# Chris10M/Ev2Hands

Measured on AMD Instinct MI355X. Metric: event-windows/sec at B=256 N=2048 (f16x2), higher is better.
Workload: dtype f32 (each f32 operand split into 2 fp16 planes with per-window power-of-two range scaling, 3 plane products per MAC on the f16 MFMA, f32 accumulate); 1 GPU; TEHNet.forward+MANO both hands, B=256/GPU N=2048 C=4 fp32, E-clouds, random-init 342-key checkpoint, synthetic MANO-shaped assets; global_batch=256, points=2048, channels=4, precision=f16x2, forwards_in_flight=1, world_size_seen=1, parallelism=batch-shard x1

## Files before the change

### ev2hands_amd/csrc/sa_mlp_bf16.hip

```cpp
#include <algorithm>
#include <cmath>
#include <cstdlib>
#include <type_traits>
#include "planes.hpp"
#include "ev2hands_hip.h"

namespace {

struct SaBP {
    const float* P1; int ldp;
    const float4* pts4;
    const float4* ctr4;
    const int32_t* gidx;
    const float4* W1x;
    const char* W2s; const float* b2;
    const char* W3s; const float* b3;
    float* out; int ldo;
    int B, Npts, S, K;
    int S_total, s_off;
    int nblk;
    const int32_t* cnt; int cnt_ld;
    float u2, u3;
    int per_xcd;
    const float* p1_scale; const unsigned* p1_amax;
    float w1x_norm, dmax, w2_norm, b2_max;
    unsigned* out_amax;
    const int32_t* nn_idx; const float* nn_w; int N;
    int ncols; int relu_out; float* out_cm; size_t out_cm_stride;
    const float* feat; int ldf; const float* W1f; int ldw1f; const float* b1; int nfeat;
    const unsigned* feat_amax; float w1f_norm, b1_max, u1f, u1x;
    float a1f, a1x, a1b;
    int spg;
    float* xyz_out; int xyz_ld;
    int t_bf16, out_bf16;
    float* row16_scale; float w3_norm, b3_max;
};

#ifdef EV2H_SAB_TIMELINE
__device__ long long g_sab_timeline[256];
#define STAMP(i) do { if (dbgw && strip == dbg_strip) g_sab_timeline[(i)] = __builtin_amdgcn_s_memtime(); } while (0)
#else
#define STAMP(i) do { } while (0)
#endif
constexpr int SAB_WAVES = 8;
constexpr int SAB_THREADS = SAB_WAVES * 64;

// ... 5 lines not shown
    static constexpr int REM = C2 % 32;
    static constexpr int M_LAST = REM == 0 ? 2 : (REM <= 16 ? 1 : 2);
    static constexpr int C2P = 32 * (T2 - 1) + 16 * M_LAST;
    static constexpr int T3 = C3 / 32;
    static constexpr int NC1 = C1 / 32;
    static constexpr int RS2 = NPL * 64 + 16;
    static constexpr int RS3 = NPL * C2P * 2 + 16;
    static constexpr int TB2 = T2 * 32 * RS2;
    static constexpr int TB3 = 32 * RS3;
    static constexpr int SB2W = F16 ? SAB_WAVES * T2 * 32 * 4 : 0;
    static constexpr int RSA = (NS == 3) ? 112 : 80;
    static constexpr int W1B = (NS == 1 || NS == 4) ? C1 * 32 : F16 ? C1 * RSA + SAB_WAVES * C1 * 4 : C1 * RSA + C1 * 4;
    static constexpr int REC_SLOTS = 64;
    static constexpr int REC = F16 ? REC_SLOTS * 4 : 0;
    static constexpr int SMALL_NOREC = W1B + T2 * 32 * 4 + 16 + SB2W;
    static constexpr int SMALL = SMALL_NOREC + REC;
    static constexpr int tile_bytes(int cpt, int upt) { return ((cpt * TB2 > upt * TB3 ? cpt * TB2 : upt * TB3) + 1023) / 1024 * 1024; }
    static constexpr bool fits(int n) { return NC1 % n == 0 && T3 % n == 0 && 2 * tile_bytes(n, n) + SMALL <= 158 * 1024; }
    static constexpr int CPT = fits(2) ? 2 : 1, UPT = CPT;
    static constexpr int TILE = tile_bytes(CPT, UPT);
    static constexpr int LDS_BYTES = 2 * TILE + SMALL;
    static constexpr int RES_W = (NC1 * TB2 + T3 * TB3 + 1023) / 1024 * 1024;
    static constexpr int RES_LDS_BYTES = RES_W + SMALL;
    static constexpr bool FITS_RESIDENT = RES_LDS_BYTES <= 160 * 1024 && C1 >= 64;
    static constexpr bool PACK4 = (NS == 2) && REM >= 1 && REM <= 4;
};

template <int C1, int C2, int C3, int NS, bool RES, int MODE>
constexpr int sab_min_waves() {
    return (NS == 4 && RES && MODE == 3 && 2 * SaBCfg<C1, C2, C3, NS>::RES_LDS_BYTES <= 160 * 1024) ? 4 : 2;
}
template <int C1, int C2, int C3, int NS, bool RES, int MODE = 0>
__global__ __launch_bounds__(SAB_THREADS, (sab_min_waves<C1, C2, C3, NS, RES, MODE>())) void sa_mlp_max_bf16_kernel(SaBP p) {
    constexpr int WV = SAB_WAVES;
    constexpr bool ROWS = MODE == 1 || MODE == 2, DIRECT = MODE == 2;
    static_assert(!(RES && ROWS), "the row-output variants stream their tiles");
    constexpr bool L1M = (NS == 1 || NS == 4) && !ROWS;
    constexpr bool L1F = (NS == 2 || NS == 3) && MODE == 3;
    constexpr bool L2PIPE = !ROWS && (NS == 1 || NS == 4) && (C1 / 32) % 2 == 0;
    constexpr bool H2FUSE = NS != 3;
    constexpr bool FRAG_PIPE = (NS != 3);
    using Cfg = SaBCfg<C1, C2, C3, NS>;
    using PL = Planes<NS>;
    constexpr int NPL = Cfg::NPL;
    constexpr bool F16 = Cfg::F16;
    constexpr int T2 = Cfg::T2, T3 = Cfg::T3, NC1 = Cfg::NC1, RS2 = Cfg::RS2, RS3 = Cfg::RS3, C2P = Cfg::C2P;
// ... 62 lines not shown
            }
        } else {
            for (int i = tid; i < C1; i += WV * 64) {
                const float4 w = p.W1x[i];
                float* d = reinterpret_cast<float*>(sW1xT) + (i >> 2) * 12 + (i & 3);
                d[0] = w.x; d[4] = w.y; d[8] = w.z;
            }
        }
    }
    for (int i = tid; i < T2 * 32; i += WV * 64) sb2[i] = p.b2[i] / p.u2;
    float* sbw = F16 ? reinterpret_cast<float*>(smem + WBYTES + Cfg::W1B + T2 * 32 * 4 + 16) + wave * (T2 * 32) : sb2;

    auto dma_tile = [&](const char* src, char* dst, int bytes) {
        for (int off = wave * 1024; off < bytes; off += WV * 1024) {
            if (off + lane * 16 < bytes)
                __builtin_amdgcn_global_load_lds((const __attribute__((address_space(1))) void*)(src + off + lane * 16),
                                                 (__attribute__((address_space(3))) void*)(dst + off), 16, 0, 0);
        }
    };
    constexpr int CPT = RES ? 1 : Cfg::CPT, UPT = RES ? 1 : Cfg::UPT;
    auto dma_w2 = [&](int step, char* dst) { dma_tile(p.W2s + (size_t)step * CPT * Cfg::TB2, dst, CPT * Cfg::TB2); };
    auto dma_w3 = [&](int step, char* dst) { dma_tile(p.W3s + (size_t)step * UPT * Cfg::TB3, dst, UPT * Cfg::TB3); };

    int buf = 0;
    if constexpr (RES && F16) {
        if (tid < Cfg::REC_SLOTS) reinterpret_cast<unsigned*>(smem + WBYTES + Cfg::SMALL_NOREC)[tid] = 0u;
    }
    if constexpr (RES) {
        dma_tile(p.W2s, smem, NC1 * Cfg::TB2);
        dma_tile(p.W3s, smem + NC1 * Cfg::TB2, T3 * Cfg::TB3);
    } else {
        dma_w2(0, wt0);
    }
    asm volatile("s_waitcnt vmcnt(0)" ::: "memory");
    __syncthreads();

    const int xcd = blockIdx.x & 7, slot = blockIdx.x >> 3, nbx = p.nblk >> 3;
    const int g_end = RES ? min(ngroups, (xcd + 1) * p.per_xcd) : ngroups;
  const int spg = (RES || ROWS) ? 1 : max(1, __builtin_amdgcn_readfirstlane(p.spg)), sw = wave % spg;
  for (int g = (RES ? xcd * p.per_xcd + slot * WV : (spg > 1 ? L * (WV / spg) + wave / spg : L * WV)) + wave * (RES || spg == 1); RES ? g < g_end : true;
       g += nbx * WV) {
    const bool valid = g < ngroups;
    const int gg = valid ? g : ngroups - 1;
    const int b = gg / p.S;
    const size_t gf = ROWS ? (size_t)gg : (size_t)b * p.S_total + p.s_off + (gg - b * p.S);
    float mrun[T3];
#pragma unroll
    for (int u = 0; u < T3; ++u) mrun[u] = -INFINITY;

    float4 ctr = make_float4(0.f, 0.f, 0.f, 0.f);
    const int32_t* gi = nullptr;
    if constexpr (!ROWS) { ctr = p.ctr4[gf]; gi = p.gidx + gf * p.K + sw * 32; }
    const int row0 = ROWS ? (gg - b * p.S) * 32 : 0;
    unsigned am = 0u;
    constexpr bool C2ONE = NS == 4 && !ROWS;
    float s1 = 1.f, c2 = p.u2, c3 = C2ONE ? p.u3 * p.u2 : p.u3;
    float so = 1.f;
    float b1s_f = 1.f, b1s_x = 1.f, b1s_b = 1.f;
    const bool fform = fmode || (L1M && hasfeat);
    if constexpr (F16) {
        if (fform && p.feat_amax) {
            const float bnd = __fmaf_rn(p.w1f_norm, __uint_as_float(p.feat_amax[b]), p.b1_max) + p.w1x_norm * p.dmax;
            s1 = f16x2_scale(__float_as_uint(bnd));
            float s2 = f16x2_scale(__float_as_uint(__fmaf_rn(p.w2_norm, bnd, p.b2_max)));
            if constexpr (C2ONE) { s1 = fminf(s1, p.u2 * s2); s2 = s1 * pow2_inverse(p.u2); }
            c2 = p.u2 * s2 * pow2_inverse(s1);
            c3 = p.u3 * pow2_inverse(s2);
        } else if (!fform && p.p1_amax) {
            float a1 = __uint_as_float(p.p1_amax[b]);
            if constexpr (DIRECT) {
                if (NS == 4 && p.t_bf16) s1 = p.row16_scale[b];
                else { s1 = f16x2_scale(p.p1_amax[b]); a1 *= s1; }
            }
            else s1 = p.p1_scale[b];
            const float inv_s1 = pow2_inverse(s1);
            const float bh1 = a1 + s1 * (p.w1x_norm * p.dmax);
            const float bh2 = __fmaf_rn(p.w2_norm, bh1 * inv_s1, p.b2_max);
            float s2 = f16x2_scale(__float_as_uint(bh2));
            c2 = p.u2 * s2 * inv_s1;
            c3 = p.u3 * pow2_inverse(s2);
            if constexpr (C2ONE) {
                s2 = s1 * pow2_inverse(p.u2);
                c3 = (s2 * bh2 <= 65504.f) ? p.u3 * pow2_inverse(s2) : __uint_as_float(0x7fc00000u);
            }
        }
        s1 = __uint_as_float(__builtin_amdgcn_readfirstlane(__float_as_uint(s1)));
        c2 = __uint_as_float(__builtin_amdgcn_readfirstlane(__float_as_uint(c2)));
        c3 = __uint_as_float(__builtin_amdgcn_readfirstlane(__float_as_uint(c3)));
        if constexpr (ROWS && NS == 4) {
            if (p.out_bf16) {
                const float bound2 = 32768.f * (c3 / p.u3);
                so = f16x2_scale(__float_as_uint(__fmaf_rn(p.w3_norm, bound2, p.b3_max)));
                so = __uint_as_float(__builtin_amdgcn_readfirstlane(__float_as_uint(so)));
                if (lane == 0 && valid && row0 == 0) p.row16_scale[b] = so;
            }
        }
        for (int i = lane; i < T2 * 32; i += 64) sbw[i] = sb2[i] * s1;
        if constexpr (L1F) {
            if (fmode) for (int i = lane; i < C1; i += 64) sb1w[i] = p.b1[i] * s1;
        }
        if constexpr (L1M) { b1s_f = s1 * p.a1f; b1s_x = s1 * p.a1x; b1s_b = s1 * p.a1b; }
    }
    int my_strips = ROWS ? 1 : p.K >> 5;
    if (!ROWS && p.cnt) my_strips = min(my_strips, max(1, (p.cnt[gf * p.cnt_ld] + 31) >> 5));
    if (spg > 1) my_strips = (valid && sw < my_strips) ? 1 : 0;
    int nstrips = my_strips;
    if constexpr (!RES && !ROWS) {
        int* s_strips = reinterpret_cast<int*>(smem + WBYTES + Cfg::W1B + T2 * 32 * 4);
        if (tid == 0) *s_strips = 1;
        __syncthreads();
        if (lane == 0) atomicMax(s_strips, my_strips);
        __syncthreads();
        nstrips = *s_strips;
    }

#ifdef EV2H_SAB_TIMELINE
    const bool dbgw = (blockIdx.x == 300 && tid == 0);
    const int dbg_strip = nstrips > 1 ? 1 : 0;
#endif
    constexpr bool XPF = !ROWS && NS != 3;
    f32x4 raw[4];
    int idx_cur = 0, idx_nxt = 0;
    float4 q_cur = make_float4(0.f, 0.f, 0.f, 0.f), f0_cur = q_cur, f1_cur = q_cur;
    if constexpr (XPF) {
        idx_cur = gi[l31];
        q_cur = p.pts4[(size_t)b * p.Npts + idx_cur];
        if (hasfeat) {
            const float4* fr = reinterpret_cast<const float4*>(p.feat + ((size_t)b * p.Npts + idx_cur) * p.ldf);
            f0_cur = fr[0]; f1_cur = fr[1];
        }
    }
    for (int strip = 0; strip < nstrips; ++strip) {
        STAMP(0);
        if constexpr (!RES) {
            if (strip >= my_strips) {
                for (int c = 0; c < NC1; ++c) {
                    char* nxt = buf ? wt0 : wt1;
                    if (c % CPT == 0) { if (c + CPT < NC1) dma_w2(c / CPT + 1, nxt); else dma_w3(0, nxt); }
                    if (c % CPT == CPT - 1) { asm volatile("s_waitcnt vmcnt(0)" ::: "memory"); __syncthreads(); buf ^= 1; }
                }
                for (int u = 0; u < T3; ++u) {
                    char* nxt = buf ? wt0 : wt1;
                    if (u % UPT == 0) { if (u + UPT < T3) dma_w3(u / UPT + 1, nxt); else if (strip + 1 < nstrips) dma_w2(0, nxt); }
                    if (u % UPT == UPT - 1) { asm volatile("s_waitcnt vmcnt(0)" ::: "memory"); __syncthreads(); buf ^= 1; }
                }
                continue;
            }
        }
        float dx = 0.f, dy = 0.f, dz = 0.f;
        auto qi = [&](int j4) { return 2 * j4 + half; };
        const float4* prow = nullptr;
        const float4* trow[3] = {nullptr, nullptr, nullptr};
        float tw[3] = {0.f, 0.f, 0.f};
        u32x4 b1f = {0u, 0u, 0u, 0u};
        u32x4 b1g = {0u, 0u, 0u, 0u};
        float cj = 1.f;
        f32x4 trw[ROWS ? 3 : 1][4];
        auto fetch = [&](int c) {
#pragma unroll
            for (int j = 0; j < ((ROWS && !DIRECT) ? 3 : 1); ++j)
#pragma unroll
                for (int j4 = 0; j4 < 4; ++j4) {
                    if constexpr ((NS == 1 || NS == 4) && DIRECT) {
                        if (p.t_bf16) {
                            const uint2 h = *reinterpret_cast<const uint2*>(reinterpret_cast<const char*>(trow[j]) + (size_t)(c * 32 + 4 * qi(j4)) * 2);
                            if constexpr (NS == 1) {
// ... 15 lines not shown
#pragma unroll
                for (int e = 0; e < 4; ++e)
                    raw[j4][e] = DIRECT ? ((F16 && !(NS == 4 && p.t_bf16)) ? trw[0][j4][e] * s1 : trw[0][j4][e])
                                        : __fmaf_rn(tw[2], trw[ROWS ? 2 : 0][j4][e], __fmaf_rn(tw[1], trw[ROWS ? 1 : 0][j4][e], __fmul_rn(tw[0], trw[0][j4][e])));
        };
        if constexpr (DIRECT) {
            trow[0] = ((NS == 1 || NS == 4) && p.t_bf16)
                          ? reinterpret_cast<const float4*>(reinterpret_cast<const char*>(p.P1) + ((size_t)b * p.N + min(row0 + l31, p.N - 1)) * p.ldp * 2)
                          : reinterpret_cast<const float4*>(p.P1 + ((size_t)b * p.N + min(row0 + l31, p.N - 1)) * p.ldp);
            fetch(0);
            blend();
        } else if constexpr (ROWS) {
            const size_t gr = ((size_t)b * p.N + min(row0 + l31, p.N - 1)) * 3;
#pragma unroll
            for (int j = 0; j < 3; ++j) {
                trow[j] = reinterpret_cast<const float4*>(p.P1 + ((size_t)b * p.Npts + p.nn_idx[gr + j]) * p.ldp);
                tw[j] = p.nn_w[gr + j];
            }
            fetch(0);
            blend();
        } else {
            const int idx = XPF ? idx_cur : gi[strip * 32 + l31];
            const float4 q = XPF ? q_cur : p.pts4[(size_t)b * p.Npts + idx];
            if constexpr (XPF) idx_nxt = (strip + 1 < my_strips) ? gi[(strip + 1) * 32 + l31] : idx_cur;
            dx = __fsub_rn(q.x, ctr.x); dy = __fsub_rn(q.y, ctr.y); dz = __fsub_rn(q.z, ctr.z);
            if constexpr (F16 && !L1M) { if (!fmode) { dx *= s1; dy *= s1; dz *= s1; } }
            if (fmode) {
                if constexpr (L1F && NS == 3) {
                    const float4* fr = reinterpret_cast<const float4*>(p.feat + ((size_t)b * p.Npts + idx) * p.ldf);
                    const float4 fa = fr[0], fb = fr[1];
                    const float v[8] = {fa.x, fa.y, fa.z, fa.w, fb.x, dx, dy, dz};
#pragma unroll
                    for (int w = 0; w < 4; ++w) {
                        unsigned o[3];
                        split_planes<3>(v[2 * w], v[2 * w + 1], o);
                        b1f[w] = half ? o[1] : o[0];
                        b1g[w] = half ? o[2] : o[0];
                    }
                }
                if constexpr (L1F && F16) {
                    float v[8] = {f0_cur.x, f0_cur.y, f0_cur.z, f0_cur.w, f1_cur.x, dx, dy, dz};
                    const float af = fmaxf(fmaxf(fmaxf(fabsf(v[0]), fabsf(v[1])), fmaxf(fabsf(v[2]), fabsf(v[3]))), fabsf(v[4]));
                    const float ax = fmaxf(fmaxf(fabsf(v[5]), fabsf(v[6])), fabsf(v[7]));
                    const float kap = fminf(f16x2_scale(__float_as_uint(af)) * (1.f / p.u1f), f16x2_scale(__float_as_uint(ax)) * (1.f / p.u1x));
                    const float sgf = kap * p.u1f, sgx = kap * p.u1x;
                    cj = s1 * pow2_inverse(kap);
#pragma unroll
                    for (int j = 0; j < 5; ++j) v[j] *= sgf;
#pragma unroll
                    for (int j = 5; j < 8; ++j) v[j] *= sgx;
#pragma unroll
                    for (int w = 0; w < 4; ++w) {
                        unsigned o[2];
                        split_planes<2>(v[2 * w], v[2 * w + 1], o);
                        b1f[w] = half ? o[1] : o[0];
                    }
                }
            } else if constexpr (L1M) {
                float f[8];
#pragma unroll
                for (int j = 0; j < 8; ++j) f[j] = 0.f;
                if (hasfeat) {
                    f[0] = f0_cur.x; f[1] = f0_cur.y; f[2] = f0_cur.z; f[3] = f0_cur.w; f[4] = f1_cur.x;
                    if constexpr (F16) {
#pragma unroll
                        for (int j = 0; j < 5; ++j) f[j] *= b1s_f;
                    }
                } else {
                    prow = reinterpret_cast<const float4*>(p.P1 + ((size_t)b * p.Npts + idx) * p.ldp);
                    if (strip == 0) {
#pragma unroll
                        for (int j4 = 0; j4 < 4; ++j4) raw[j4] = *reinterpret_cast<const f32x4*>(prow + qi(j4));
                    }
                }
                auto lo_of = [](float x) {
                    if constexpr (F16) return x - (float)(_Float16)x;
                    else return x - __uint_as_float(__builtin_bit_cast(unsigned, __builtin_convertvector(f32x2{x, 0.f}, bf16x2)) << 16);
                };
                const float ex = F16 ? dx * b1s_x : dx, ey = F16 ? dy * b1s_x : dy, ez = F16 ? dz * b1s_x : dz;
                const float va[8] = {f[0], f[1], f[2], f[3], f[4], lo_of(ex), lo_of(ey), lo_of(ez)};
                const float vb[8] = {ex, ey, ez, F16 ? (hasfeat ? b1s_b : 0.f) : 1.f, lo_of(f[0]), lo_of(f[1]), lo_of(f[2]), lo_of(f[3])};
#pragma unroll
                for (int w = 0; w < 4; ++w) {
                    unsigned o[1];
                    split_planes<NS>(half ? vb[2 * w] : va[2 * w], half ? vb[2 * w + 1] : va[2 * w + 1], o);
                    b1f[w] = o[0];
                }
            } else {
                prow = reinterpret_cast<const float4*>(p.P1 + ((size_t)b * p.Npts + idx) * p.ldp);
                if (!XPF || strip == 0) {
#pragma unroll
                    for (int j4 = 0; j4 < 4; ++j4) raw[j4] = *reinterpret_cast<const f32x4*>(prow + qi(j4));
                }
            }
        }
        auto layer1 = [&](int c) {
            f32x16 acc;
            if constexpr (L1F && NS == 3) {
#pragma unroll
                for (int q = 0; q < 4; ++q) {
                    const f32x4 bv = *reinterpret_cast<const f32x4*>(sb1w + 32 * c + 8 * q + 4 * half);
#pragma unroll
                    for (int e = 0; e < 4; ++e) acc[4 * q + e] = bv[e];
                }
                const char* ar = smem + WBYTES + (32 * c + l31) * Cfg::RSA + half * 16;
                const u32x4 a0 = *reinterpret_cast<const u32x4*>(ar), a1 = *reinterpret_cast<const u32x4*>(ar + 32), a2 = *reinterpret_cast<const u32x4*>(ar + 64);
                acc = mfma_planes<3>(a2, b1g, acc);
                acc = mfma_planes<3>(a1, b1f, acc);
                return mfma_planes<3>(a0, b1f, acc);
            } else if constexpr (L1F) {
#pragma unroll
                for (int r = 0; r < 16; ++r) acc[r] = 0.f;
                const char* ar = smem + WBYTES + (32 * c + l31) * Cfg::RSA + half * 16;
// ... 111 lines not shown
            if constexpr (FRAG_PIPE) ld2(0, fa[0][0], fa[0][1]);
#pragma unroll
            for (int pr = 0; pr < T2; ++pr) {
                const int m0 = (2 * pr) / T2, t0 = (2 * pr) % T2, m1 = (2 * pr + 1) / T2, t1 = (2 * pr + 1) % T2;
                if constexpr (FRAG_PIPE) {
                    if (pr + 1 < T2) ld2(pr + 1, fa[(pr + 1) & 1][0], fa[(pr + 1) & 1][1]);
                    __builtin_amdgcn_sched_barrier(0);
                } else {
                    ld2(pr, fa[pr & 1][0], fa[pr & 1][1]);
                }
                u32x4 (&a0)[NPL] = fa[pr & 1][0];
                u32x4 (&a1)[NPL] = fa[pr & 1][1];
#pragma unroll
                for (int j = 0; j < PL::NPROD; ++j) {
                    if (!(Cfg::PACK4 && t0 == T2 - 1 && PL::A[j] == 1)) h2[t0] = mfma_planes<NS>(a0[PL::A[j]], bp[m0][PL::B[j]], h2[t0]);
                    if (!(Cfg::PACK4 && t1 == T2 - 1 && PL::A[j] == 1)) h2[t1] = mfma_planes<NS>(a1[PL::A[j]], bp[m1][PL::B[j]], h2[t1]);
                }
                if constexpr (FRAG_PIPE) __builtin_amdgcn_sched_barrier(0);
                between(pr);
            }
        };
        auto l2_dma = [&](int c) {
            if constexpr (!RES) {
                char* nxt = buf ? wt0 : wt1;
                if (c % CPT == 0) { if (c + CPT < NC1) dma_w2(c / CPT + 1, nxt); else dma_w3(0, nxt); }
            }
        };
        auto l2_sync = [&](int c) {
            STAMP(4 + 4 * c);
            if constexpr (!RES) {
                if (c % CPT == CPT - 1) {
                    asm volatile("s_waitcnt vmcnt(0)" ::: "memory");
                    __syncthreads();
                    buf ^= 1;
                }
            }
            STAMP(5 + 4 * c);
        };
        u32x4 bpA[2][NPL];
        if constexpr (!L2PIPE) {
#pragma unroll 1
            for (int c = 0; c < NC1; ++c) {
                STAMP(2 + 4 * c);
                char* cur = RES ? smem + c * Cfg::TB2 : (buf ? wt1 : wt0) + (c % CPT) * Cfg::TB2;
                l2_dma(c);
#pragma unroll
                for (int j4 = 0; j4 < 4; ++j4) finish_slice(c, j4, bpA);
                if constexpr (ROWS) {
                    if (c + 1 < NC1) fetch(c + 1);
                } else if (!L1M && !fmode && c + 1 < NC1) {
#pragma unroll
                    for (int j4 = 0; j4 < 4; ++j4) raw[j4] = *reinterpret_cast<const f32x4*>(prow + (c + 1) * 8 + qi(j4));
                }
                STAMP(3 + 4 * c);
                mfma_groups(cur, bpA, [](int) {});
                if constexpr (ROWS) {
                    if (c + 1 < NC1) blend();
                }
                if constexpr (L1F) {
                    if (fmode && c + 1 < NC1) d1 = layer1(c + 1);
                }
                if constexpr (L1M) {
                    if (c + 1 < NC1) {
                        d1 = layer1(c + 1);
                        if (!hasfeat && c + 2 < NC1) {
#pragma unroll
                            for (int j4 = 0; j4 < 4; ++j4) raw[j4] = *reinterpret_cast<const f32x4*>(prow + (c + 2) * 8 + qi(j4));
                        }
                    }
                }
                l2_sync(c);
            }
        } else {
            u32x4 bpB[2][NPL];
            const bool vtab = !L1M && !fmode;
#pragma unroll
            for (int j4 = 0; j4 < 4; ++j4) {
                finish_slice(0, j4, bpA);
                if (vtab) raw[j4] = *reinterpret_cast<const f32x4*>(prow + 8 + qi(j4));
            }
            auto l2_step = [&](int c, u32x4 (&bc)[2][NPL], u32x4 (&bn)[2][NPL]) {
                STAMP(2 + 4 * c);
                char* cur = RES ? smem + c * Cfg::TB2 : (buf ? wt1 : wt0) + (c % CPT) * Cfg::TB2;
                l2_dma(c);
                const bool more = c + 1 < NC1;
                if (more) {
                    if constexpr (L1F) { if (fmode) d1 = layer1(c + 1); }
                    if constexpr (L1M) {
                        d1 = layer1(c + 1);
                        if (!hasfeat && c + 2 < NC1) {
#pragma unroll
                            for (int j4 = 0; j4 < 4; ++j4) raw[j4] = *reinterpret_cast<const f32x4*>(prow + (c + 2) * 8 + qi(j4));
                        }
                    }
                }
                STAMP(3 + 4 * c);
                mfma_groups(cur, bc, [&](int pr) {
                    if (more) {
#pragma unroll
                        for (int j4 = 0; j4 < 4; ++j4) {
                            if (j4 * T2 / 4 == pr) {
                                __builtin_amdgcn_sched_barrier(0);
                                finish_slice(c + 1, j4, bn);
                                if (vtab && c + 2 < NC1) raw[j4] = *reinterpret_cast<const f32x4*>(prow + (c + 2) * 8 + qi(j4));
                                __builtin_amdgcn_sched_barrier(0);
                            }
                        }
                    }
                });
                l2_sync(c);
            };
#pragma unroll 1
            for (int c = 0; c < NC1; c += 2) {
                l2_step(c, bpA, bpB);
                l2_step(c + 1, bpB, bpA);
            }
        }

        STAMP(38);
        if constexpr (XPF) {
            if (strip + 1 < my_strips) {
                q_cur = p.pts4[(size_t)b * p.Npts + idx_nxt];
                if (hasfeat) {
                    const float4* fr = reinterpret_cast<const float4*>(p.feat + ((size_t)b * p.Npts + idx_nxt) * p.ldf);
                    f0_cur = fr[0]; f1_cur = fr[1];
                } else {
                    const float4* pn = reinterpret_cast<const float4*>(p.P1 + ((size_t)b * p.Npts + idx_nxt) * p.ldp);
#pragma unroll
                    for (int j4 = 0; j4 < 4; ++j4) raw[j4] = *reinterpret_cast<const f32x4*>(pn + qi(j4));
                }
                idx_cur = idx_nxt;
            }
        }
        if constexpr (Cfg::PACK4) {
#pragma unroll
            for (int r = 0; r < 4; ++r) { h2[T2 - 1][r] += h2[T2 - 1][r + 4]; h2[T2 - 1][r + 4] = 0.f; }
        }
        u32x4 h2p[NPL][T2][2];
        auto split_half = [&](int t, int m) {
#pragma unroll
            for (int k = 4 * m; k < 4 * m + 4; ++k) {
                unsigned o[NPL];
                if constexpr (C2ONE) {
                    split_planes<NS>(h2[t][2 * k], h2[t][2 * k + 1], o);
                    o[0] = relu_pk_bf16(o[0]);
                }
                else if constexpr (F16) split_planes<NS>(relu_sat_f16(h2[t][2 * k] * c2), relu_sat_f16(h2[t][2 * k + 1] * c2), o);
                else if constexpr (NS == 1) { split_planes<NS>(h2[t][2 * k], h2[t][2 * k + 1], o); o[0] = relu_pk_bf16(o[0]); }
                else split_planes<NS>(relu_bits(h2[t][2 * k] * c2), relu_bits(h2[t][2 * k + 1] * c2), o);
#pragma unroll
// ... 8 lines not shown
                    h2p[0][T2 - 1][0][1] = half ? ph23 : h23;
                    h2p[0][T2 - 1][0][2] = half ? 0u : l01;
                    h2p[0][T2 - 1][0][3] = half ? 0u : l23;
                }
            }
        };
#pragma unroll
        for (int t = 0; t < (H2FUSE ? 1 : T2); ++t) { split_half(t, 0); split_half(t, 1); }
        STAMP(39);

        auto finish_tile = [&](int u, const f32x16& acc) {
            float mx = fmaxf(fmaxf(acc[0], acc[1]), acc[2]);
#pragma unroll
            for (int r = 3; r < 15; r += 2) mx = fmaxf(fmaxf(mx, acc[r]), acc[r + 1]);
            mx = fmaxf(mx, acc[15]);
#pragma unroll
            for (int uu = 0; uu < T3; ++uu) mrun[uu] = (uu == u) ? fmaxf(mrun[uu], mx) : mrun[uu];
        };
        constexpr int TPS = (!ROWS && (RES || UPT == 2)) ? 2 : 1;
        static_assert(T3 % TPS == 0, "layer-3 tiles are walked in pairs");
        auto l3_step = [&](int u, auto first_tag) {
            constexpr bool FIRST = decltype(first_tag)::value;
            STAMP(40 + 4 * u);
            char* cur = RES ? smem + NC1 * Cfg::TB2 + u * Cfg::TB3 : (buf ? wt1 : wt0) + (u % UPT) * Cfg::TB3;
            char* nxt = buf ? wt0 : wt1;
            if constexpr (!RES) {
                if (u % UPT == 0) {
                    const bool more_w3 = (u + UPT < T3);
                    const bool more = more_w3 || (strip + 1 < nstrips);
                    if (more_w3) dma_w3(u / UPT + 1, nxt); else if (more) dma_w2(0, nxt);
                }
            }
            float b3u = 0.f;
            if constexpr (ROWS) b3u = p.b3[32 * u + l31];
            f32x16 acc, acc1;
#pragma unroll
            for (int r = 0; r < 16; ++r) { acc[r] = 0.f; acc1[r] = 0.f; }
            const char* pb = cur + l31 * RS3 + (8 * half) * 2;
            constexpr int NG3 = 2 * (T2 - 1) + Cfg::M_LAST;
            auto ld3 = [&](int g, u32x4 (&x)[NPL], u32x4 (&x1)[TPS == 2 ? NPL : 1]) {
#pragma unroll
                for (int s = 0; s < NPL; ++s) {
                    x[s] = *reinterpret_cast<const u32x4*>(pb + s * (C2P * 2) + (16 * g) * 2);
                    if constexpr (TPS == 2) x1[s] = *reinterpret_cast<const u32x4*>(pb + Cfg::TB3 + s * (C2P * 2) + (16 * g) * 2);
                }
            };
            u32x4 fw[2][NPL], fw1[2][TPS == 2 ? NPL : 1];
            if constexpr (FRAG_PIPE) ld3(0, fw[0], fw1[0]);
#pragma unroll
            for (int t = 0; t < T2; ++t) {
#pragma unroll
                for (int m = 0; m < 2; ++m) {
// ... 63 lines not shown
                            if (ocm) ocm[pt] = o;
                            am = max(am, abs_bits(o));
                        }
                    }
                } else {
                    finish_tile(u, acc);
                }
            }
            STAMP(42 + 4 * u);
            if constexpr (!RES) {
                if ((u + TPS - 1) % UPT == UPT - 1) {
                    asm volatile("s_waitcnt vmcnt(0)" ::: "memory");
                    __syncthreads();
                    buf ^= 1;
                }
            }
            STAMP(43 + 4 * u);
        };
        if constexpr (H2FUSE) l3_step(0, std::true_type{});
#pragma unroll 1
        for (int u = H2FUSE ? TPS : 0; u < T3; u += TPS) l3_step(u, std::false_type{});
        STAMP(37);
    }
    if constexpr (!ROWS && !RES) {
        if (spg > 1) {
            float* smax = reinterpret_cast<float*>(smem);
#pragma unroll
            for (int u = 0; u < T3; ++u) {
                const float v = fmaxf(mrun[u], __shfl_xor(mrun[u], 32, 64));
                if (half == 0) smax[wave * C3 + 32 * u + l31] = v;
            }
            __syncthreads();
            if (sw == 0) {
#pragma unroll
                for (int u = 0; u < T3; ++u) {
                    float v = smax[wave * C3 + 32 * u + l31];
                    for (int k = 1; k < spg; ++k) v = fmaxf(v, smax[(wave + k) * C3 + 32 * u + l31]);
                    mrun[u] = v;
                }
            }
        }
    }
    if constexpr (!ROWS) {
#pragma unroll
        for (int u = 0; u < T3; ++u) {
            const float v = fmaxf(mrun[u], __shfl_xor(mrun[u], 32, 64));
            if (valid && half == 0 && sw == 0) {
                float o = fmaxf(v * c3 + p.b3[32 * u + l31], 0.f);
                if constexpr (C2ONE) o = (c3 == c3) ? o : c3;
                p.out[gf * p.ldo + 32 * u + l31] = o;
                am = max(am, __float_as_uint(o));
            }
        }
    }
    if constexpr (!ROWS) {
        if (p.xyz_out && valid && sw == 0 && lane < 8)
            p.xyz_out[gf * p.xyz_ld + lane] = lane == 0 ? ctr.x : lane == 1 ? ctr.y : lane == 2 ? ctr.z : 0.f;
    }
    if constexpr (F16) {
        if (p.out_amax) {
            am = wave_max_u32_dpp(am);
            char* rec = smem + WBYTES + Cfg::SMALL_NOREC;
            if constexpr (RES) {
                if (lane == 0 && am) {
                    const int slot = b - (xcd * p.per_xcd) / p.S;
                    unsigned old = 0u;
                    if (slot >= 0 && slot < Cfg::REC_SLOTS) old = atomicMax(reinterpret_cast<unsigned*>(rec) + slot, am);
                    if (am > old) atomicMax(&p.out_amax[b], am);
                }
            } else {
                int* sb = reinterpret_cast<int*>(rec);
                unsigned* sa = reinterpret_cast<unsigned*>(rec + 32);
                if (lane == 0) { sb[wave] = (valid && am) ? b : -1; sa[wave] = am; }
                __syncthreads();
                if (lane == 0 && valid && am) {
                    bool first = true;
                    unsigned m = am;
#pragma unroll
                    for (int w = 0; w < WV; ++w) {
                        if (sb[w] == b) { first = first && w >= wave; m = max(m, sa[w]); }
                    }
                    if (first) atomicMax(&p.out_amax[b], m);
                }
            }
        }
    }
    if constexpr (!RES) break;
  }
}

template <int C1, int C2, int C3, int NS, int MODE = 0>
int launch_sab(SaBP p, hipStream_t st) {
    using Cfg = SaBCfg<C1, C2, C3, NS>;
    static const bool streamed_only = getenv("EV2H_SA_STREAMED") != nullptr;
    if constexpr (Cfg::FITS_RESIDENT) {
        if (!streamed_only) {
            static PerDevice wg_slot{};
            std::atomic<int>& wg = wg_slot.cur();
            int wg_per_cu = wg.load(std::memory_order_acquire);
            if (!wg_per_cu) {
                auto k = sa_mlp_max_bf16_kernel<C1, C2, C3, NS, true, MODE>;
                EV2H_CHECK_HIP(hipFuncSetAttribute(reinterpret_cast<const void*>(k), hipFuncAttributeMaxDynamicSharedMemorySize, Cfg::RES_LDS_BYTES));
                int n = 0;
                EV2H_CHECK_HIP(hipOccupancyMaxActiveBlocksPerMultiprocessor(&n, k, SAB_THREADS, Cfg::RES_LDS_BYTES));
                wg_per_cu = n > 0 ? n : 1;
                wg.store(wg_per_cu, std::memory_order_release);
            }
            const int ngroups = p.B * p.S;
            const int want = 256 * wg_per_cu;
            p.per_xcd = ceil_div(ceil_div(ngroups, 8), SAB_WAVES) * SAB_WAVES;
            p.nblk = 8 * std::min(want / 8, ceil_div(p.per_xcd, SAB_WAVES));
            sa_mlp_max_bf16_kernel<C1, C2, C3, NS, true, MODE><<<p.nblk, SAB_THREADS, Cfg::RES_LDS_BYTES, st>>>(p);
            EV2H_CHECK_LAUNCH();
            return EV2H_OK;
        }
    }
    static PerDevice attr_set{};
    EV2H_ONCE_PER_DEVICE(attr_set,
        EV2H_CHECK_HIP(hipFuncSetAttribute(reinterpret_cast<const void*>(sa_mlp_max_bf16_kernel<C1, C2, C3, NS, false, MODE>),
                                           hipFuncAttributeMaxDynamicSharedMemorySize, Cfg::LDS_BYTES)););
    {
        const int spg = p.K / 32;
        p.spg = 1;
        if ((spg == 2 || spg == 4) && p.nblk < 256 && SAB_WAVES * C3 * 4 <= 2 * Cfg::TILE) {
            p.spg = spg;
            p.nblk = ceil_div(p.B * p.S, SAB_WAVES / spg);
        }
    }
    sa_mlp_max_bf16_kernel<C1, C2, C3, NS, false, MODE><<<p.nblk, SAB_THREADS, Cfg::LDS_BYTES, st>>>(p);
    EV2H_CHECK_LAUNCH();
    return EV2H_OK;
}

template <int NS, int MODE = 0>
int dispatch_sab(const SaBP& p, int c1, int c2, int c3, hipStream_t st) {
    if constexpr (MODE == 0) {
        if (p.feat) return dispatch_sab<NS, 3>(p, c1, c2, c3, st);
    }
    if (c1 == 32 && c2 == 32 && c3 == 64) return launch_sab<32, 32, 64, NS, MODE>(p, st);
    if (c1 == 64 && c2 == 64 && c3 == 128) return launch_sab<64, 64, 128, NS, MODE>(p, st);
    if (c1 == 64 && c2 == 96 && c3 == 128) return launch_sab<64, 96, 128, NS, MODE>(p, st);
    if (c1 == 128 && c2 == 128 && c3 == 256) return launch_sab<128, 128, 256, NS, MODE>(p, st);
    if (c1 == 128 && c2 == 196 && c3 == 256) return launch_sab<128, 196, 256, NS, MODE>(p, st);
    ev2h_set_error("ev2h_sa_mlp_max: unsupported MLP widths %d-%d-%d", c1, c2, c3);
    return EV2H_ERR_ARG;
}

}

#ifdef EV2H_SAB_TIMELINE
extern "C" int ev2h_sab_timeline_read(long long* host) {
    return (int)hipMemcpyFromSymbol(host, HIP_SYMBOL(g_sab_timeline), sizeof(long long) * 256);
// ... 142 lines not shown
```

Baseline: 21370 event-windows/s.

## Make streamed SA MLP kernel persistent with cross-group weight and gather prefetch

When the streamed (non-resident) set-abstraction MLP grid would exceed one wave of workgroups, the launch now uses a persistent grid of 256×occupancy blocks. Each block walks its XCD-local range of groups and prefetches the next group's header, strip count, first gather indices, point rows and first W2 tile while finishing the current group. Per-group strip counts are exchanged through double-buffered LDS bytes, which replaces the two syncthreads/atomic reduction. Biases are cached in extra LDS, the per-wave bias rescale is skipped when the scale is unchanged, and kernel args are read through the kernarg pointer. The cost is extra LDS, more register pressure and more complex control flow, and the change can slightly lower occupancy.

```diff
diff --git a/ev2hands_amd/csrc/sa_mlp_bf16.hip b/ev2hands_amd/csrc/sa_mlp_bf16.hip
--- a/ev2hands_amd/csrc/sa_mlp_bf16.hip
+++ b/ev2hands_amd/csrc/sa_mlp_bf16.hip
@@ -22,6 +22,7 @@
     const int32_t* cnt; int cnt_ld;
     float u2, u3;
     int per_xcd;
+    int pers;
     const float* p1_scale; const unsigned* p1_amax;
     float w1x_norm, dmax, w2_norm, b2_max;
     unsigned* out_amax;
@@ -73,6 +74,7 @@
     static constexpr int LDS_BYTES = 2 * TILE + SMALL;
     static constexpr int RES_W = (NC1 * TB2 + T3 * TB3 + 1023) / 1024 * 1024;
     static constexpr int RES_LDS_BYTES = RES_W + SMALL;
+    static constexpr int SAB_XTR = (C3 + C1) * 4;
     static constexpr bool FITS_RESIDENT = RES_LDS_BYTES <= 160 * 1024 && C1 >= 64;
     static constexpr bool PACK4 = (NS == 2) && REM >= 1 && REM <= 4;
 };
@@ -181,6 +183,11 @@
     auto dma_w2 = [&](int step, char* dst) { dma_tile(p.W2s + (size_t)step * CPT * Cfg::TB2, dst, CPT * Cfg::TB2); };
     auto dma_w3 = [&](int step, char* dst) { dma_tile(p.W3s + (size_t)step * UPT * Cfg::TB3, dst, UPT * Cfg::TB3); };
 
+    constexpr bool PERS = !RES && !ROWS;
+    const bool pers = PERS && p.pers;
+    if constexpr (PERS) {
+        if (pers && (int)(blockIdx.x & 7) * p.per_xcd + (int)(blockIdx.x >> 3) * WV >= min(p.B * p.S, ((int)(blockIdx.x & 7) + 1) * p.per_xcd)) return;
+    }
     int buf = 0;
     if constexpr (RES && F16) {
         if (tid < Cfg::REC_SLOTS) reinterpret_cast<unsigned*>(smem + WBYTES + Cfg::SMALL_NOREC)[tid] = 0u;
@@ -191,86 +198,144 @@
     } else {
         dma_w2(0, wt0);
     }
+    const int xcd = blockIdx.x & 7, slot = blockIdx.x >> 3, nbx = RES ? p.nblk >> 3 : (int)(gridDim.x >> 3);
+    const int g_end = (RES || pers) ? min(ngroups, (xcd + 1) * p.per_xcd) : ngroups;
+    const int spg = (RES || ROWS) ? 1 : max(1, __builtin_amdgcn_readfirstlane(p.spg)), sw = wave % spg;
+    int g = ((RES || pers) ? xcd * p.per_xcd + slot * WV : (spg > 1 ? L * (WV / spg) + wave / spg : L * WV)) + wave * (RES || spg == 1);
+    constexpr bool fform = fmode || (L1M && hasfeat);
+    typedef const SaBP __attribute__((address_space(4)))* KargP;
+    KargP pk = (KargP)__builtin_amdgcn_kernarg_segment_ptr();
+#define HA(f) (PERS ? pk->f : p.f)
+    struct Head { bool valid; int b; size_t gf; };
+    auto head_of = [&](int g_) {
+        Head h;
+        h.valid = g_ < ngroups;
+        const int gg_ = h.valid ? g_ : ngroups - 1;
+        h.b = gg_ / HA(S);
+        h.gf = ROWS ? (size_t)gg_ : (size_t)h.b * HA(S_total) + HA(s_off) + (gg_ - h.b * HA(S));
+        return h;
+    };
+    auto strips_of = [&](Head h) {
+        int n = ROWS ? 1 : HA(K) >> 5;
+        if (!ROWS && HA(cnt)) n = min(n, max(1, (HA(cnt)[h.gf * HA(cnt_ld)] + 31) >> 5));
+        if (spg > 1) n = (h.valid && sw < n) ? 1 : 0;
+        return n;
+    };
+    float4 ctr_n = make_float4(0.f, 0.f, 0.f, 0.f);
+    int strips_n = 0;
+    unsigned amax_n = 0u;
+    float scale_n = 1.f;
+    auto load_head = [&](Head h) {
+        ctr_n = HA(ctr4)[h.gf];
+        strips_n = strips_of(h);
+        if constexpr (F16) {
+            if (fform && HA(feat_amax)) amax_n = HA(feat_amax)[h.b];
+            else if (!fform && HA(p1_amax)) { amax_n = HA(p1_amax)[h.b]; scale_n = HA(p1_scale)[h.b]; }
+        }
+    };
+    unsigned char* s_strips = reinterpret_cast<unsigned char*>(smem + WBYTES + Cfg::W1B + T2 * 32 * 4);
+    int par = 0;
+    float* sb3 = reinterpret_cast<float*>(smem + Cfg::LDS_BYTES);
+    float* sb1u = sb3 + C3;
+    const Head h0 = head_of(g);
+    bool hc_valid = h0.valid; int hc_b = h0.b; size_t hc_gf = h0.gf;
+    if constexpr (PERS) {
+        for (int i = tid; i < C3; i += WV * 64) sb3[i] = p.b3[i];
+        if constexpr (L1F && F16) {
+            if (fmode) for (int i = tid; i < C1; i += WV * 64) sb1u[i] = p.b1[i];
+        }
+        load_head(h0);
+        if (lane == 0) s_strips[wave] = (unsigned char)strips_n;
+    }
     asm volatile("s_waitcnt vmcnt(0)" ::: "memory");
     __syncthreads();
 
-    const int xcd = blockIdx.x & 7, slot = blockIdx.x >> 3, nbx = p.nblk >> 3;
-    const int g_end = RES ? min(ngroups, (xcd + 1) * p.per_xcd) : ngroups;
-  const int spg = (RES || ROWS) ? 1 : max(1, __builtin_amdgcn_readfirstlane(p.spg)), sw = wave % spg;
-  for (int g = (RES ? xcd * p.per_xcd + slot * WV : (spg > 1 ? L * (WV / spg) + wave / spg : L * WV)) + wave * (RES || spg == 1); RES ? g < g_end : true;
-       g += nbx * WV) {
-    const bool valid = g < ngroups;
+    f32x4 raw[4];
+    int idx_cur = 0, idx_nxt = 0;
+    float4 q_cur = make_float4(0.f, 0.f, 0.f, 0.f), f0_cur = q_cur, f1_cur = q_cur;
+    bool pref = false;
+    float s1_prev = __uint_as_float(0x7fc00000u);
+  for (; RES ? g < g_end : true; g += nbx * WV) {
+    if constexpr (PERS) asm volatile("" : "+s"(pk));
+    const bool valid = PERS ? hc_valid : g < ngroups;
     const int gg = valid ? g : ngroups - 1;
-    const int b = gg / p.S;
-    const size_t gf = ROWS ? (size_t)gg : (size_t)b * p.S_total + p.s_off + (gg - b * p.S);
+    const int b = PERS ? hc_b : gg / HA(S);
+    const size_t gf = PERS ? hc_gf : ROWS ? (size_t)gg : (size_t)b * HA(S_total) + HA(s_off) + (gg - b * HA(S));
     float mrun[T3];
 #pragma unroll
     for (int u = 0; u < T3; ++u) mrun[u] = -INFINITY;
 
     float4 ctr = make_float4(0.f, 0.f, 0.f, 0.f);
     const int32_t* gi = nullptr;
-    if constexpr (!ROWS) { ctr = p.ctr4[gf]; gi = p.gidx + gf * p.K + sw * 32; }
-    const int row0 = ROWS ? (gg - b * p.S) * 32 : 0;
+    if constexpr (!ROWS) { if constexpr (PERS) ctr = ctr_n; else ctr = HA(ctr4)[gf]; gi = HA(gidx) + gf * HA(K) + sw * 32; }
+    const int my_strips_pers = strips_n;
+    const unsigned hamax = amax_n;
+    const float hscale = scale_n;
+    const bool more_oct = pers && (g - wave + nbx * WV < g_end);
+    bool hn_valid = valid; int hn_b = b; size_t hn_gf = gf;
+    if constexpr (PERS) {
+        if (more_oct) { const Head h = head_of(g + nbx * WV); load_head(h); hn_valid = h.valid; hn_b = h.b; hn_gf = h.gf; }
+    }
+    const int row0 = ROWS ? (gg - b * HA(S)) * 32 : 0;
     unsigned am = 0u;
     constexpr bool C2ONE = NS == 4 && !ROWS;
-    float s1 = 1.f, c2 = p.u2, c3 = C2ONE ? p.u3 * p.u2 : p.u3;
+    float s1 = 1.f, c2 = HA(u2), c3 = C2ONE ? HA(u3) * HA(u2) : HA(u3);
     float so = 1.f;
     float b1s_f = 1.f, b1s_x = 1.f, b1s_b = 1.f;
-    const bool fform = fmode || (L1M && hasfeat);
     if constexpr (F16) {
-        if (fform && p.feat_amax) {
-            const float bnd = __fmaf_rn(p.w1f_norm, __uint_as_float(p.feat_amax[b]), p.b1_max) + p.w1x_norm * p.dmax;
+        if (fform && HA(feat_amax)) {
+            const float bnd = __fmaf_rn(HA(w1f_norm), __uint_as_float(PERS ? hamax : HA(feat_amax)[b]), HA(b1_max)) + HA(w1x_norm) * HA(dmax);
             s1 = f16x2_scale(__float_as_uint(bnd));
-            float s2 = f16x2_scale(__float_as_uint(__fmaf_rn(p.w2_norm, bnd, p.b2_max)));
-            if constexpr (C2ONE) { s1 = fminf(s1, p.u2 * s2); s2 = s1 * pow2_inverse(p.u2); }
-            c2 = p.u2 * s2 * pow2_inverse(s1);
-            c3 = p.u3 * pow2_inverse(s2);
-        } else if (!fform && p.p1_amax) {
-            float a1 = __uint_as_float(p.p1_amax[b]);
+            float s2 = f16x2_scale(__float_as_uint(__fmaf_rn(HA(w2_norm), bnd, HA(b2_max))));
+            if constexpr (C2ONE) { s1 = fminf(s1, HA(u2) * s2); s2 = s1 * pow2_inverse(HA(u2)); }
+            c2 = HA(u2) * s2 * pow2_inverse(s1);
+            c3 = HA(u3) * pow2_inverse(s2);
+        } else if (!fform && HA(p1_amax)) {
+            float a1 = __uint_as_float(PERS ? hamax : HA(p1_amax)[b]);
             if constexpr (DIRECT) {
-                if (NS == 4 && p.t_bf16) s1 = p.row16_scale[b];
-                else { s1 = f16x2_scale(p.p1_amax[b]); a1 *= s1; }
-            }
-            else s1 = p.p1_scale[b];
+                if (NS == 4 && HA(t_bf16)) s1 = HA(row16_scale)[b];
+                else { s1 = f16x2_scale(HA(p1_amax)[b]); a1 *= s1; }
+            }
+            else s1 = PERS ? hscale : HA(p1_scale)[b];
             const float inv_s1 = pow2_inverse(s1);
-            const float bh1 = a1 + s1 * (p.w1x_norm * p.dmax);
-            const float bh2 = __fmaf_rn(p.w2_norm, bh1 * inv_s1, p.b2_max);
+            const float bh1 = a1 + s1 * (HA(w1x_norm) * HA(dmax));
+            const float bh2 = __fmaf_rn(HA(w2_norm), bh1 * inv_s1, HA(b2_max));
             float s2 = f16x2_scale(__float_as_uint(bh2));
-            c2 = p.u2 * s2 * inv_s1;
-            c3 = p.u3 * pow2_inverse(s2);
+            c2 = HA(u2) * s2 * inv_s1;
+            c3 = HA(u3) * pow2_inverse(s2);
             if constexpr (C2ONE) {
-                s2 = s1 * pow2_inverse(p.u2);
-                c3 = (s2 * bh2 <= 65504.f) ? p.u3 * pow2_inverse(s2) : __uint_as_float(0x7fc00000u);
+                s2 = s1 * pow2_inverse(HA(u2));
+                c3 = (s2 * bh2 <= 65504.f) ? HA(u3) * pow2_inverse(s2) : __uint_as_float(0x7fc00000u);
             }
         }
         s1 = __uint_as_float(__builtin_amdgcn_readfirstlane(__float_as_uint(s1)));
         c2 = __uint_as_float(__builtin_amdgcn_readfirstlane(__float_as_uint(c2)));
         c3 = __uint_as_float(__builtin_amdgcn_readfirstlane(__float_as_uint(c3)));
         if constexpr (ROWS && NS == 4) {
-            if (p.out_bf16) {
-                const float bound2 = 32768.f * (c3 / p.u3);
-                so = f16x2_scale(__float_as_uint(__fmaf_rn(p.w3_norm, bound2, p.b3_max)));
+            if (HA(out_bf16)) {
+                const float bound2 = 32768.f * (c3 / HA(u3));
+                so = f16x2_scale(__float_as_uint(__fmaf_rn(HA(w3_norm), bound2, HA(b3_max))));
                 so = __uint_as_float(__builtin_amdgcn_readfirstlane(__float_as_uint(so)));
-                if (lane == 0 && valid && row0 == 0) p.row16_scale[b] = so;
-            }
-        }
-        for (int i = lane; i < T2 * 32; i += 64) sbw[i] = sb2[i] * s1;
-        if constexpr (L1F) {
-            if (fmode) for (int i = lane; i < C1; i += 64) sb1w[i] = p.b1[i] * s1;
-        }
-        if constexpr (L1M) { b1s_f = s1 * p.a1f; b1s_x = s1 * p.a1x; b1s_b = s1 * p.a1b; }
-    }
-    int my_strips = ROWS ? 1 : p.K >> 5;
-    if (!ROWS && p.cnt) my_strips = min(my_strips, max(1, (p.cnt[gf * p.cnt_ld] + 31) >> 5));
-    if (spg > 1) my_strips = (valid && sw < my_strips) ? 1 : 0;
+                if (lane == 0 && valid && row0 == 0) HA(row16_scale)[b] = so;
+            }
+        }
+        if (!PERS || s1 != s1_prev) {
+            for (int i = lane; i < T2 * 32; i += 64) sbw[i] = sb2[i] * s1;
+            if constexpr (L1F) {
+                if (fmode) for (int i = lane; i < C1; i += 64) sb1w[i] = (PERS ? sb1u[i] : HA(b1)[i]) * s1;
+            }
+            s1_prev = s1;
+        }
+        if constexpr (L1M) { b1s_f = s1 * HA(a1f); b1s_x = s1 * HA(a1x); b1s_b = s1 * HA(a1b); }
+    }
+    const int my_strips = PERS ? my_strips_pers : strips_of(Head{valid, b, gf});
     int nstrips = my_strips;
-    if constexpr (!RES && !ROWS) {
-        int* s_strips = reinterpret_cast<int*>(smem + WBYTES + Cfg::W1B + T2 * 32 * 4);
-        if (tid == 0) *s_strips = 1;
-        __syncthreads();
-        if (lane == 0) atomicMax(s_strips, my_strips);
-        __syncthreads();
-        nstrips = *s_strips;
+    if constexpr (PERS) {
+        const uint2 sv = *reinterpret_cast<const uint2*>(s_strips + par * 8);
+        const unsigned s_lo = __builtin_amdgcn_readfirstlane(sv.x), s_hi = __builtin_amdgcn_readfirstlane(sv.y);
+        nstrips = 1;
+#pragma unroll
+        for (int w = 0; w < 4; ++w) nstrips = max(nstrips, (int)max((s_lo >> (8 * w)) & 0xffu, (s_hi >> (8 * w)) & 0xffu));
     }
 
 #ifdef EV2H_SAB_TIMELINE
@@ -278,10 +343,7 @@
     const int dbg_strip = nstrips > 1 ? 1 : 0;
 #endif
     constexpr bool XPF = !ROWS && NS != 3;
-    f32x4 raw[4];
-    int idx_cur = 0, idx_nxt = 0;
-    float4 q_cur = make_float4(0.f, 0.f, 0.f, 0.f), f0_cur = q_cur, f1_cur = q_cur;
-    if constexpr (XPF) {
+    if (XPF && !pref) {
         idx_cur = gi[l31];
         q_cur = p.pts4[(size_t)b * p.Npts + idx_cur];
         if (hasfeat) {
@@ -294,13 +356,16 @@
         if constexpr (!RES) {
             if (strip >= my_strips) {
                 for (int c = 0; c < NC1; ++c) {
-                    char* nxt = buf ? wt0 : wt1;
+                    char* nxt = smem + (buf ^ 1) * Cfg::TILE;
                     if (c % CPT == 0) { if (c + CPT < NC1) dma_w2(c / CPT + 1, nxt); else dma_w3(0, nxt); }
                     if (c % CPT == CPT - 1) { asm volatile("s_waitcnt vmcnt(0)" ::: "memory"); __syncthreads(); buf ^= 1; }
                 }
+                if constexpr (PERS) {
+                    if (more_oct && strip + 1 == nstrips && lane == 0) s_strips[(par ^ 1) * 8 + wave] = (unsigned char)strips_n;
+                }
                 for (int u = 0; u < T3; ++u) {
-                    char* nxt = buf ? wt0 : wt1;
-                    if (u % UPT == 0) { if (u + UPT < T3) dma_w3(u / UPT + 1, nxt); else if (strip + 1 < nstrips) dma_w2(0, nxt); }
+                    char* nxt = smem + (buf ^ 1) * Cfg::TILE;
+                    if (u % UPT == 0) { if (u + UPT < T3) dma_w3(u / UPT + 1, nxt); else if (strip + 1 < nstrips || more_oct) dma_w2(0, nxt); }
                     if (u % UPT == UPT - 1) { asm volatile("s_waitcnt vmcnt(0)" ::: "memory"); __syncthreads(); buf ^= 1; }
                 }
                 continue;
@@ -362,7 +427,7 @@
         } else {
             const int idx = XPF ? idx_cur : gi[strip * 32 + l31];
             const float4 q = XPF ? q_cur : p.pts4[(size_t)b * p.Npts + idx];
-            if constexpr (XPF) idx_nxt = (strip + 1 < my_strips) ? gi[(strip + 1) * 32 + l31] : idx_cur;
+            if constexpr (XPF) idx_nxt = (strip + 1 < my_strips) ? gi[(strip + 1) * 32 + l31] : (more_oct ? p.gidx[hn_gf * p.K + l31] : idx_cur);
             dx = __fsub_rn(q.x, ctr.x); dy = __fsub_rn(q.y, ctr.y); dz = __fsub_rn(q.z, ctr.z);
             if constexpr (F16 && !L1M) { if (!fmode) { dx *= s1; dy *= s1; dz *= s1; } }
             if (fmode) {
@@ -408,7 +473,7 @@
                     }
                 } else {
                     prow = reinterpret_cast<const float4*>(p.P1 + ((size_t)b * p.Npts + idx) * p.ldp);
-                    if (strip == 0) {
+                    if (strip == 0 && !pref) {
 #pragma unroll
                         for (int j4 = 0; j4 < 4; ++j4) raw[j4] = *reinterpret_cast<const f32x4*>(prow + qi(j4));
                     }
@@ -428,7 +493,7 @@
                 }
             } else {
                 prow = reinterpret_cast<const float4*>(p.P1 + ((size_t)b * p.Npts + idx) * p.ldp);
-                if (!XPF || strip == 0) {
+                if (!XPF || (strip == 0 && !pref)) {
 #pragma unroll
                     for (int j4 = 0; j4 < 4; ++j4) raw[j4] = *reinterpret_cast<const f32x4*>(prow + qi(j4));
                 }
@@ -586,7 +651,7 @@
         };
         auto l2_dma = [&](int c) {
             if constexpr (!RES) {
-                char* nxt = buf ? wt0 : wt1;
+                char* nxt = smem + (buf ^ 1) * Cfg::TILE;
                 if (c % CPT == 0) { if (c + CPT < NC1) dma_w2(c / CPT + 1, nxt); else dma_w3(0, nxt); }
             }
         };
@@ -606,7 +671,7 @@
 #pragma unroll 1
             for (int c = 0; c < NC1; ++c) {
                 STAMP(2 + 4 * c);
-                char* cur = RES ? smem + c * Cfg::TB2 : (buf ? wt1 : wt0) + (c % CPT) * Cfg::TB2;
+                char* cur = RES ? smem + c * Cfg::TB2 : (smem + buf * Cfg::TILE) + (c % CPT) * Cfg::TB2;
                 l2_dma(c);
 #pragma unroll
                 for (int j4 = 0; j4 < 4; ++j4) finish_slice(c, j4, bpA);
@@ -645,7 +710,7 @@
             }
             auto l2_step = [&](int c, u32x4 (&bc)[2][NPL], u32x4 (&bn)[2][NPL]) {
                 STAMP(2 + 4 * c);
-                char* cur = RES ? smem + c * Cfg::TB2 : (buf ? wt1 : wt0) + (c % CPT) * Cfg::TB2;
+                char* cur = RES ? smem + c * Cfg::TB2 : (smem + buf * Cfg::TILE) + (c % CPT) * Cfg::TB2;
                 l2_dma(c);
                 const bool more = c + 1 < NC1;
                 if (more) {
@@ -682,14 +747,18 @@
         }
 
         STAMP(38);
+        if constexpr (PERS) {
+            if (more_oct && strip + 1 == nstrips && lane == 0) s_strips[(par ^ 1) * 8 + wave] = (unsigned char)strips_n;
+        }
         if constexpr (XPF) {
-            if (strip + 1 < my_strips) {
-                q_cur = p.pts4[(size_t)b * p.Npts + idx_nxt];
+            if (strip + 1 < my_strips || more_oct) {
+                const int bx = (strip + 1 < my_strips) ? b : hn_b;
+                q_cur = p.pts4[(size_t)bx * p.Npts + idx_nxt];
                 if (hasfeat) {
-                    const float4* fr = reinterpret_cast<const float4*>(p.feat + ((size_t)b * p.Npts + idx_nxt) * p.ldf);
+                    const float4* fr = reinterpret_cast<const float4*>(p.feat + ((size_t)bx * p.Npts + idx_nxt) * p.ldf);
                     f0_cur = fr[0]; f1_cur = fr[1];
                 } else {
-                    const float4* pn = reinterpret_cast<const float4*>(p.P1 + ((size_t)b * p.Npts + idx_nxt) * p.ldp);
+                    const float4* pn = reinterpret_cast<const float4*>(p.P1 + ((size_t)bx * p.Npts + idx_nxt) * p.ldp);
 #pragma unroll
                     for (int j4 = 0; j4 < 4; ++j4) raw[j4] = *reinterpret_cast<const f32x4*>(pn + qi(j4));
                 }
@@ -744,12 +813,12 @@
         auto l3_step = [&](int u, auto first_tag) {
             constexpr bool FIRST = decltype(first_tag)::value;
             STAMP(40 + 4 * u);
-            char* cur = RES ? smem + NC1 * Cfg::TB2 + u * Cfg::TB3 : (buf ? wt1 : wt0) + (u % UPT) * Cfg::TB3;
-            char* nxt = buf ? wt0 : wt1;
+            char* cur = RES ? smem + NC1 * Cfg::TB2 + u * Cfg::TB3 : (smem + buf * Cfg::TILE) + (u % UPT) * Cfg::TB3;
+            char* nxt = smem + (buf ^ 1) * Cfg::TILE;
             if constexpr (!RES) {
                 if (u % UPT == 0) {
                     const bool more_w3 = (u + UPT < T3);
-                    const bool more = more_w3 || (strip + 1 < nstrips);
+                    const bool more = more_w3 || (strip + 1 < nstrips) || more_oct;
                     if (more_w3) dma_w3(u / UPT + 1, nxt); else if (more) dma_w2(0, nxt);
                 }
             }
@@ -859,6 +928,7 @@
         for (int u = H2FUSE ? TPS : 0; u < T3; u += TPS) l3_step(u, std::false_type{});
         STAMP(37);
     }
+    if constexpr (PERS) asm volatile("" : "+s"(pk));
     if constexpr (!ROWS && !RES) {
         if (spg > 1) {
             float* smax = reinterpret_cast<float*>(smem);
@@ -883,27 +953,27 @@
         for (int u = 0; u < T3; ++u) {
             const float v = fmaxf(mrun[u], __shfl_xor(mrun[u], 32, 64));
             if (valid && half == 0 && sw == 0) {
-                float o = fmaxf(v * c3 + p.b3[32 * u + l31], 0.f);
+                float o = fmaxf(v * c3 + (PERS ? sb3[32 * u + l31] : HA(b3)[32 * u + l31]), 0.f);
                 if constexpr (C2ONE) o = (c3 == c3) ? o : c3;
-                p.out[gf * p.ldo + 32 * u + l31] = o;
+                HA(out)[gf * HA(ldo) + 32 * u + l31] = o;
                 am = max(am, __float_as_uint(o));
             }
         }
     }
     if constexpr (!ROWS) {
-        if (p.xyz_out && valid && sw == 0 && lane < 8)
-            p.xyz_out[gf * p.xyz_ld + lane] = lane == 0 ? ctr.x : lane == 1 ? ctr.y : lane == 2 ? ctr.z : 0.f;
+        if (HA(xyz_out) && valid && sw == 0 && lane < 8)
+            HA(xyz_out)[gf * HA(xyz_ld) + lane] = lane == 0 ? ctr.x : lane == 1 ? ctr.y : lane == 2 ? ctr.z : 0.f;
     }
     if constexpr (F16) {
-        if (p.out_amax) {
+        if (HA(out_amax)) {
             am = wave_max_u32_dpp(am);
             char* rec = smem + WBYTES + Cfg::SMALL_NOREC;
             if constexpr (RES) {
                 if (lane == 0 && am) {
-                    const int slot = b - (xcd * p.per_xcd) / p.S;
+                    const int slot = b - (xcd * HA(per_xcd)) / HA(S);
                     unsigned old = 0u;
                     if (slot >= 0 && slot < Cfg::REC_SLOTS) old = atomicMax(reinterpret_cast<unsigned*>(rec) + slot, am);
-                    if (am > old) atomicMax(&p.out_amax[b], am);
+                    if (am > old) atomicMax(&HA(out_amax)[b], am);
                 }
             } else {
                 int* sb = reinterpret_cast<int*>(rec);
@@ -917,12 +987,18 @@
                     for (int w = 0; w < WV; ++w) {
                         if (sb[w] == b) { first = first && w >= wave; m = max(m, sa[w]); }
                     }
-                    if (first) atomicMax(&p.out_amax[b], m);
-                }
-            }
-        }
-    }
-    if constexpr (!RES) break;
+                    if (first) atomicMax(&HA(out_amax)[b], m);
+                }
+            }
+        }
+    }
+#undef HA
+    if constexpr (!RES) {
+        if (!more_oct) break;
+        par ^= 1;
+        pref = XPF;
+        hc_valid = hn_valid; hc_b = hn_b; hc_gf = hn_gf;
+    }
   }
 }
 
@@ -952,10 +1028,18 @@
             return EV2H_OK;
         }
     }
-    static PerDevice attr_set{};
-    EV2H_ONCE_PER_DEVICE(attr_set,
-        EV2H_CHECK_HIP(hipFuncSetAttribute(reinterpret_cast<const void*>(sa_mlp_max_bf16_kernel<C1, C2, C3, NS, false, MODE>),
-                                           hipFuncAttributeMaxDynamicSharedMemorySize, Cfg::LDS_BYTES)););
+    static PerDevice wg_slot_s{};
+    std::atomic<int>& wgs = wg_slot_s.cur();
+    int wg_per_cu = wgs.load(std::memory_order_acquire);
+    if (!wg_per_cu) {
+        auto k = sa_mlp_max_bf16_kernel<C1, C2, C3, NS, false, MODE>;
+        static_assert(Cfg::LDS_BYTES + Cfg::SAB_XTR <= 160 * 1024, "LDS");
+        EV2H_CHECK_HIP(hipFuncSetAttribute(reinterpret_cast<const void*>(k), hipFuncAttributeMaxDynamicSharedMemorySize, Cfg::LDS_BYTES + Cfg::SAB_XTR));
+        int n = 0;
+        EV2H_CHECK_HIP(hipOccupancyMaxActiveBlocksPerMultiprocessor(&n, k, SAB_THREADS, Cfg::LDS_BYTES + Cfg::SAB_XTR));
+        wg_per_cu = n > 0 ? n : 1;
+        wgs.store(wg_per_cu, std::memory_order_release);
+    }
     {
         const int spg = p.K / 32;
         p.spg = 1;
@@ -964,7 +1048,14 @@
             p.nblk = ceil_div(p.B * p.S, SAB_WAVES / spg);
         }
     }
-    sa_mlp_max_bf16_kernel<C1, C2, C3, NS, false, MODE><<<p.nblk, SAB_THREADS, Cfg::LDS_BYTES, st>>>(p);
+    int grid = p.nblk;
+    p.pers = 0;
+    if (p.spg == 1 && p.nblk > 256 * wg_per_cu) {
+        p.pers = 1;
+        p.per_xcd = ceil_div(ceil_div(p.B * p.S, 8), SAB_WAVES) * SAB_WAVES;
+        grid = 256 * wg_per_cu;
+    }
+    sa_mlp_max_bf16_kernel<C1, C2, C3, NS, false, MODE><<<grid, SAB_THREADS, Cfg::LDS_BYTES + Cfg::SAB_XTR, st>>>(p);
     EV2H_CHECK_LAUNCH();
     return EV2H_OK;
 }
```

New measurement: 21670 event-windows/s, median of 6. 1.01x the previous value.
